# ZJULiHongxin/HRNet-Hand-Pose-Estimation

Measured on AMD Instinct MI355X. Metric: images/sec fwd+bwd pose_hrnet_w32 256x256 bs=64/GPU, higher is better.
Workload: dtype bf16; 1 GPU; pose_hrnet_w32 256x256 bf16 fwd+HeatmapLoss+bwd+Adam training step, batch 64/GPU, synthetic RHD-shaped crops, random-init weights; global_batch=64, parallelism=dp1

## Files before the change

### hrnet-hand-pose-estimation_amd/csrc/loss.hip

```cpp
#include "common.h"

namespace {

__device__ __forceinline__ float block_sum(float v, float* red) {
  v = wave_sum64(v);
  const int w = threadIdx.x >> 6;
  if ((threadIdx.x & 63) == 0) red[w] = v;
  __syncthreads();
  float s = 0.f;
  for (int k = 0; k < (int)(blockDim.x >> 6); ++k) s += red[k];
  __syncthreads();
  return s;
}

__device__ __forceinline__ float block_max(float v, float* red) {
#pragma unroll
  for (int o = 32; o > 0; o >>= 1) v = fmaxf(v, __shfl_xor(v, o, 64));
  const int w = threadIdx.x >> 6;
  if ((threadIdx.x & 63) == 0) red[w] = v;
  __syncthreads();
  float m = red[0];
  for (int k = 1; k < (int)(blockDim.x >> 6); ++k) m = fmaxf(m, red[k]);
  __syncthreads();
  return m;
// ... 189 lines not shown
    if (inference_style) {
      u = (float)(idx % W);
      v = (float)(idx / W);
      if (!(mx > 0.f)) u = v = 0.f;
    } else {
      u = (float)(idx % H);
      v = (float)(idx / H);
    }
    preds[blockIdx.x * 2] = u;
    preds[blockIdx.x * 2 + 1] = v;
    if (maxvals) maxvals[blockIdx.x] = mx;
  }
}

__global__ __launch_bounds__(256) void joints_loss_fwd_kernel(const float* pred, const float* gt,
                                                              const float* vis, float* loss, int B, int K) {
  __shared__ float red[4];
  float s = 0.f, sv = 0.f;
  for (int i = threadIdx.x; i < B * K; i += 256) {
    const float dx = pred[2 * i] - gt[2 * i], dy = pred[2 * i + 1] - gt[2 * i + 1];
    const float nrm = sqrtf(dx * dx + dy * dy);
    const float w = vis ? vis[i] : 1.f;
    s = fmaf(nrm, w, s);
    sv += w;
  }
  s = block_sum(s, red);
  sv = block_sum(sv, red);
  if (threadIdx.x == 0) loss[0] = vis ? s / fmaxf(1.f, sv) : s / (float)K;
}

__global__ __launch_bounds__(256) void joints_loss_bwd_kernel(const float* pred, const float* gt,
                                                              const float* vis, const float* gout,
                                                              float* dpred, int B, int K) {
  __shared__ float red[4];
  float sv = 0.f;
  if (vis)
    for (int i = threadIdx.x; i < B * K; i += 256) sv += vis[i];
  sv = block_sum(sv, red);
  const float denom = vis ? fmaxf(1.f, sv) : (float)K;
  const float g = gout[0] / denom;
  for (int i = threadIdx.x; i < B * K; i += 256) {
    const float dx = pred[2 * i] - gt[2 * i], dy = pred[2 * i + 1] - gt[2 * i + 1];
    const float nrm = sqrtf(dx * dx + dy * dy);
    const float w = (vis ? vis[i] : 1.f) * g;
    dpred[2 * i] = nrm > 0.f ? w * dx / nrm : 0.f;
    dpred[2 * i + 1] = nrm > 0.f ? w * dy / nrm : 0.f;
  }
}

__global__ __launch_bounds__(256) void joints3d_loss_fwd_kernel(const float* __restrict__ pred,
                                                                const float* __restrict__ gt,
                                                                float* __restrict__ loss, int B, int K) {
  __shared__ double part[256];
  double s = 0.0;
  for (int i = threadIdx.x; i < B * K; i += 256) {
    const double dx = (double)gt[3 * i] - (double)pred[3 * i], dy = (double)gt[3 * i + 1] - (double)pred[3 * i + 1],
                 dz = (double)gt[3 * i + 2] - (double)pred[3 * i + 2];
    s += sqrt(dx * dx + dy * dy + dz * dz);
  }
  part[threadIdx.x] = s;
  __syncthreads();
  if (threadIdx.x == 0) {
    double total = 0.0;
    for (int i = 0; i < 256; ++i) total += part[i];
    loss[0] = (float)(total / (double)K);
  }
}

__global__ __launch_bounds__(256) void joints3d_loss_bwd_kernel(const float* __restrict__ pred,
                                                                const float* __restrict__ gt,
                                                                const float* __restrict__ gout,
                                                                float* __restrict__ dpred, int n, int K) {
  const double g = (double)gout[0] / (double)K;
  for (int i = blockIdx.x * 256 + threadIdx.x; i < n; i += gridDim.x * 256) {
    const double dx = (double)pred[3 * i] - (double)gt[3 * i], dy = (double)pred[3 * i + 1] - (double)gt[3 * i + 1],
                 dz = (double)pred[3 * i + 2] - (double)gt[3 * i + 2];
    const double nrm = sqrt(dx * dx + dy * dy + dz * dz);
    dpred[3 * i] = nrm == 0.0 ? 0.f : (float)(g * dx / nrm);
    dpred[3 * i + 1] = nrm == 0.0 ? 0.f : (float)(g * dy / nrm);
    dpred[3 * i + 2] = nrm == 0.0 ? 0.f : (float)(g * dz / nrm);
  }
}

__global__ __launch_bounds__(256) void adam_kernel(float* p, const float* g, float* m, float* v,
                                                   long long n, float lr, float b1, float b2, float eps,
                                                   float wd, float bc1, float bc2_sqrt, float gscale) {
  for (long long i = (long long)blockIdx.x * blockDim.x + threadIdx.x; i < n;
       i += (long long)gridDim.x * blockDim.x) {
    float gi = g[i] * gscale;
    const float pi = p[i];
    gi = fmaf(wd, pi, gi);
    const float mi = b1 * m[i] + (1.f - b1) * gi;
    const float vi = b2 * v[i] + (1.f - b2) * gi * gi;
    m[i] = mi;
    v[i] = vi;
    const float denom = sqrtf(vi) / bc2_sqrt + eps;
    p[i] = pi - (lr / bc1) * (mi / denom);
  }
}

constexpr int kHandJoints = 21;
constexpr int kStructThreads = 256;

__device__ __forceinline__ double hand_scale(double (&x)[kHandJoints][2]) {
  const double wx = x[0][0], wy = x[0][1];
#pragma unroll
  for (int j = 0; j < kHandJoints; ++j) {
    x[j][0] -= wx;
    x[j][1] -= wy;
  }
  const double ux = x[9][0] - x[0][0], uy = x[9][1] - x[0][1];
  const double s = sqrt(ux * ux + uy * uy);
#pragma unroll
  for (int j = 0; j < kHandJoints; ++j) {
    x[j][0] /= s;
    x[j][1] /= s;
  }
  return s;
}

__device__ __forceinline__ void hand_grad_store(double (&g)[kHandJoints][2], const double (&x)[kHandJoints][2],
                                                double s, int normalize, float* __restrict__ out) {
  if (normalize) {
    double gs = 0.0;
#pragma unroll
    for (int j = 0; j < kHandJoints; ++j) {
      gs += g[j][0] * x[j][0] + g[j][1] * x[j][1];
      g[j][0] /= s;
      g[j][1] /= s;
    }
    gs = -gs / s;
    const double ux = x[9][0] - x[0][0], uy = x[9][1] - x[0][1];
    const double nx = s == 0.0 ? 0.0 : ux, ny = s == 0.0 ? 0.0 : uy;
    g[9][0] += gs * nx;
    g[9][1] += gs * ny;
    g[0][0] -= gs * nx;
    g[0][1] -= gs * ny;
    double sx = 0.0, sy = 0.0;
#pragma unroll
    for (int j = 0; j < kHandJoints; ++j) {
      sx += g[j][0];
      sy += g[j][1];
    }
    g[0][0] -= sx;
    g[0][1] -= sy;
  }
#pragma unroll
  for (int j = 0; j < kHandJoints; ++j) {
    out[2 * j] = (float)g[j][0];
    out[2 * j + 1] = (float)g[j][1];
  }
}

__device__ __forceinline__ void hand_load(const float* __restrict__ p, double (&x)[kHandJoints][2]) {
#pragma unroll
  for (int j = 0; j < kHandJoints; ++j) {
    x[j][0] = (double)p[2 * j];
    x[j][1] = (double)p[2 * j + 1];
  }
}

__global__ __launch_bounds__(kStructThreads) void structure_loss_kernel(const float* __restrict__ pred,
                                                                        const float* __restrict__ gt,
                                                                        float* __restrict__ loss_bone,
                                                                        float* __restrict__ loss_angle,
                                                                        float* __restrict__ dbone,
                                                                        float* __restrict__ dangle, int B,
                                                                        int normalize, int terms) {
  __shared__ double part[2][kStructThreads];
  double sum_bone = 0.0, sum_angle = 0.0;
  for (int base = 0; base < B; base += kStructThreads) {
    const int b = base + (int)threadIdx.x;
    double lb = 0.0, la = 0.0;
    if (b < B) {
      double x[kHandJoints][2], g[kHandJoints][2];
      hand_load(pred + (size_t)b * kHandJoints * 2, x);
      const double s = normalize ? hand_scale(x) : 1.0;
      if (terms & 1) {
        double lg[kHandJoints];
        {
// ... 181 lines not shown
extern "C" int hrnet_decode_argmax(const float* hms, float* preds, float* maxvals, int BK, int H, int W,
                                   int inference_style, hr_stream_t stream) {
  HR_REQUIRE(hms && preds && BK > 0 && H > 0 && W > 0, "decode_argmax: args");
  hipLaunchKernelGGL(decode_argmax_kernel, dim3(BK), dim3(256), 0, (hipStream_t)stream, hms, preds,
                     maxvals, H, W, inference_style);
  return hr_check_launch("decode_argmax");
}

extern "C" int hrnet_joints_loss_fwd(const float* pred, const float* gt, const float* vis, float* loss,
                                     int B, int K, hr_stream_t stream) {
  HR_REQUIRE(pred && gt && loss && B > 0 && K > 0, "joints_loss_fwd: args");
  hipLaunchKernelGGL(joints_loss_fwd_kernel, dim3(1), dim3(256), 0, (hipStream_t)stream, pred, gt, vis,
                     loss, B, K);
  return hr_check_launch("joints_loss_fwd");
}

extern "C" int hrnet_joints_loss_bwd(const float* pred, const float* gt, const float* vis,
                                     const float* gout, float* dpred, int B, int K, hr_stream_t stream) {
  HR_REQUIRE(pred && gt && gout && dpred && B > 0 && K > 0, "joints_loss_bwd: args");
  hipLaunchKernelGGL(joints_loss_bwd_kernel, dim3(1), dim3(256), 0, (hipStream_t)stream, pred, gt, vis,
                     gout, dpred, B, K);
  return hr_check_launch("joints_loss_bwd");
}

extern "C" int hrnet_joints3d_loss_fwd(const float* pred, const float* gt, float* loss, int B, int K,
                                       hr_stream_t stream) {
  HR_REQUIRE(pred && gt && loss && B > 0 && K > 0 && (long long)B * K <= (1LL << 28), "joints3d_loss_fwd: args");
  hipLaunchKernelGGL(joints3d_loss_fwd_kernel, dim3(1), dim3(256), 0, (hipStream_t)stream, pred, gt, loss, B, K);
  return hr_check_launch("joints3d_loss_fwd");
}

extern "C" int hrnet_joints3d_loss_bwd(const float* pred, const float* gt, const float* gout, float* dpred, int B,
                                       int K, hr_stream_t stream) {
  HR_REQUIRE(pred && gt && gout && dpred && B > 0 && K > 0 && (long long)B * K <= (1LL << 28),
             "joints3d_loss_bwd: args");
  const int n = B * K;
  int grid = (n + 255) / 256;
  if (grid > 1024) grid = 1024;
  hipLaunchKernelGGL(joints3d_loss_bwd_kernel, dim3((unsigned)grid), dim3(256), 0, (hipStream_t)stream, pred, gt,
                     gout, dpred, n, K);
  return hr_check_launch("joints3d_loss_bwd");
}

extern "C" int hrnet_structure_loss(const float* pred, const float* gt, float* loss_bone, float* loss_angle,
                                    float* dbone_dpred, float* dangle_dpred, int B, int K, int normalize, int terms,
                                    hr_stream_t stream) {
  HR_REQUIRE(pred && B > 0, "structure_loss: args");
  HR_REQUIRE(K == kHandJoints, "structure_loss: K must be 21 (the hand skeleton of the reference's losses)");
  HR_REQUIRE(terms >= 1 && terms <= 3, "structure_loss: terms is a mask of 1 (bone length) and 2 (joint angle)");
  HR_REQUIRE(!(terms & 1) || (gt && loss_bone), "structure_loss: the bone-length term needs gt and loss_bone");
  HR_REQUIRE(!(terms & 2) || loss_angle, "structure_loss: the joint-angle term needs loss_angle");
  hipLaunchKernelGGL(structure_loss_kernel, dim3(1), dim3(kStructThreads), 0, (hipStream_t)stream, pred, gt,
                     loss_bone, loss_angle, (terms & 1) ? dbone_dpred : nullptr, (terms & 2) ? dangle_dpred : nullptr,
                     B, normalize ? 1 : 0, terms);
  return hr_check_launch("structure_loss");
}

extern "C" int hrnet_structure_loss_bwd(const float* dbone_dpred, const float* dangle_dpred, const float* g_bone,
                                        const float* g_angle, float* dpred, int B, int K, hr_stream_t stream) {
  HR_REQUIRE(dpred && B > 0 && K == kHandJoints, "structure_loss_bwd: args");
  HR_REQUIRE((g_bone || g_angle) && (!g_bone || dbone_dpred) && (!g_angle || dangle_dpred),
             "structure_loss_bwd: an upstream gradient needs its unit gradient");
  const long long n = (long long)B * K * 2;
  long long grid = (n + 255) / 256;
  if (grid > 1024) grid = 1024;
  hipLaunchKernelGGL(structure_loss_bwd_kernel, dim3((unsigned)grid), dim3(256), 0, (hipStream_t)stream,
                     dbone_dpred, dangle_dpred, g_bone, g_angle, dpred, n);
  return hr_check_launch("structure_loss_bwd");
}

extern "C" int hrnet_adam_step(float* param, const float* grad, float* exp_avg, float* exp_avg_sq,
                               int64_t n, float lr, float beta1, float beta2, float eps,
                               float weight_decay, int step, float grad_scale, hr_stream_t stream) {
  HR_REQUIRE(param && grad && exp_avg && exp_avg_sq && n > 0 && step >= 1, "adam_step: args");
  const double bc1 = 1.0 - pow((double)beta1, (double)step);
  const double bc2 = 1.0 - pow((double)beta2, (double)step);
  long long grid = (n + 255) / 256;
  if (grid > 8192) grid = 8192;
  hipLaunchKernelGGL(adam_kernel, dim3((unsigned)grid), dim3(256), 0, (hipStream_t)stream, param, grad,
                     exp_avg, exp_avg_sq, (long long)n, lr, beta1, beta2, eps, weight_decay, (float)bc1,
                     (float)sqrt(bc2), grad_scale);
  return hr_check_launch("adam_step");
}
```

### hrnet-hand-pose-estimation_amd/lib/hipnet/net.py

```python
import torch
import torch.nn as nn

from . import _capi as C
from . import ops
from .engine import BNRec, ConvRec, Plan, Program


class HipNet(object):
    def __init__(self, module, stage_cfg, compute_dtype):
        self.module = module
        self.stage_cfg = stage_cfg
        self.compute_dtype = compute_dtype
        self.dtid = C.dtype_id(compute_dtype)
        C.lib()
        params = list(module.parameters())
        if not params or not params[0].is_cuda:
            raise RuntimeError('pose_hrnet: parameters must live on a HIP device (model.cuda()); '
                               'there is no CPU path')
        self.device = params[0].device
        self.plans = {}
        self.fwd_packed = self.bwd_packed = False
        self._flatten(params)
        self._records()

    def _flatten(self, params):
        names = {id(p): n for n, p in self.module.named_parameters()}
        self._late_ids = {id(p) for p in params if p.requires_grad and self._is_late(names.get(id(p), ''), p)}
        params = ([p for p in params if p.requires_grad and id(p) not in self._late_ids]
                  + [p for p in params if id(p) in self._late_ids] + [p for p in params if not p.requires_grad])
        self.trainable_count = sum(p.numel() for p in params if p.requires_grad)
        self.late_start = sum(p.numel() for p in params if p.requires_grad and id(p) not in self._late_ids)
        total = sum(p.numel() for p in params)
        self.flat_p = torch.empty(total, dtype=torch.float32, device=self.device)
        self.flat_g = torch.zeros(total, dtype=torch.float32, device=self.device)
        self.params = params
        self._gview = {}
        self.offsets = {}
        off = 0
        with torch.no_grad():
            for p in params:
                n = p.numel()
                self.flat_p[off:off + n].copy_(p.detach().reshape(-1).float())
                p.data = self.flat_p[off:off + n].view(p.shape)
                self._gview[id(p)] = self.flat_g[off:off + n].view(p.shape)
                self.offsets[id(p)] = (off, n)
                if p.grad is not None:
                    self._gview[id(p)].copy_(p.grad)
                    p.grad = self._gview[id(p)]
                off += n
        self.total_params = total

    def grad_of(self, p):
        return self._gview[id(p)]

    def layout(self):
        names = {id(p): n for n, p in self.module.named_parameters()}
        return [(names[id(p)],) + self.offsets[id(p)] for p in self.params if p.requires_grad]

    def param_order(self):
        return [n for n, _p in self.module.named_parameters()]

    @staticmethod
    def _is_late(name, p):
        if p.dim() != 4 or not name.startswith('stage') or not name.endswith('.weight'):
            return False
        parts = name.split('.')
        if 'fuse_layers' in parts:
            return True
        return 'branches' in parts and int(parts[parts.index('branches') + 1]) >= 2

    def is_late(self, p):
        return id(p) in self._late_ids

    def _records(self):
        self.convs, self.bns, self.bn_list, self.bias_pad = {}, {}, {}, {}
        self.bn_list = []
        skip = tuple(getattr(self.module, 'hip_skip_prefixes', ()))
        for name, m in self.module.named_modules():
            if skip and name.startswith(skip):
                continue
            if isinstance(m, nn.Conv2d):
                r = ConvRec(name, m, stem=(name == 'conv1'))
                es = torch.empty((), dtype=self.compute_dtype).element_size()
                taps = r.ks * r.ks
                nf = r.Cout_pad * (1 if r.stem else taps) * r.Cin_pad
                r.wf = torch.empty(nf * es, dtype=torch.uint8, device=self.device)
                if not r.stem:
                    r.wd = torch.empty(r.Cin_pad * taps * r.Cout_pad * es, dtype=torch.uint8, device=self.device)
                self.convs[name] = r
                if m.bias is not None:
                    self.bias_pad[name] = torch.zeros(r.Cout_pad, dtype=torch.float32, device=self.device)
            elif isinstance(m, nn.BatchNorm2d):
                b = BNRec(name, m, self.device)
                self.bns[name] = b
                self.bn_list.append(b)
        self.pack_f = self._pack_program([(r, 2 if r.stem else 0, r.wf) for r in self.convs.values()])
        self.pack_d = self._pack_program([(r, 1, r.wd) for r in self.convs.values() if r.wd is not None])

    def _pack_program(self, items):
        import ctypes
        ents = (C.HrPackEnt * len(items))()
        block = 0
        for e, item in zip(ents, items):
            r, mode, out = item[:3]
            taps = r.ks * r.ks
            if (mode == 1 and r.Cout_pad * (taps + 1) > 4864) or (mode == 0 and r.Cin * taps > 4864):
                raise ValueError('{}: {} output channels at {}x{} exceed the LDS staging of the weight packer'.format(
                    r.prefix, r.Cout, r.ks, r.ks))
            e.w, e.out = C.ptr(r.mod.weight), C.ptr(out)
            e.Cout, e.Cin, e.ks, e.Cout_pad, e.Cin_pad, e.mode = r.Cout, r.Cin, r.ks, r.Cout_pad, r.Cin_pad, mode
            if len(item) > 3:
                c0, c = item[3], item[4]
                assert r.ks == 1 and mode == 0
                e.w = r.mod.weight.data_ptr() + 4 * c0
                e.Cin, e.Cin_pad, e.ld = c, c, r.Cin
            e.block0 = block
            block += C.call('hrnet_pack_blocks', e.Cout_pad, e.Cin_pad, r.ks, mode)
        raw = bytes(ctypes.string_at(ctypes.addressof(ents), ctypes.sizeof(ents)))
        table = torch.frombuffer(bytearray(raw), dtype=torch.uint8).to(self.device)
        self._tables = getattr(self, '_tables', []) + [table]
        prog = Program()
        prog.add(ops.make(C.OP_PACK_TABLE, dtype=self.dtid, n=len(items), blocks=block, table=C.ptr(table)))
        return prog.finalize()

    def head_slices(self, crec, widths):
        key = (crec.prefix, tuple(widths))
        if getattr(self, '_head_key', None) != key:
            es = torch.empty((), dtype=self.compute_dtype).element_size()
            items, off = [], 0
            self._head_wf = []
            for c in widths:
                out = torch.empty(crec.Cout_pad * c * es, dtype=torch.uint8, device=self.device)
                self._head_wf.append(out)
                items.append((crec, 0, out, off, c))
                off += c
            self._head_pack = self._pack_program(items)
            self._head_key = key
            self._head_pack.run()
        return self._head_wf

    def pack_weights(self, for_backward):
        if not self.fwd_packed:
            self.pack_f.run()
            if getattr(self, '_head_pack', None) is not None:
                self._head_pack.run()
            for name, buf in self.bias_pad.items():
                b = self.convs[name].mod.bias
                buf[:b.numel()].copy_(b.detach())
            self.fwd_packed = True
        if for_backward and not self.bwd_packed:
            self.pack_d.run()
            self.bwd_packed = True

    def mark_weights_dirty(self):
        self.fwd_packed = self.bwd_packed = False

    MAX_PLANS_IN_FLIGHT = 4

    def plan(self, N, H, W, training, need_grad):
        key = (N, H, W, bool(training), bool(need_grad))
        pool = self.plans.setdefault(key, [])
        for p in pool:
            if not (need_grad and p.busy):
                return p
        if len(pool) >= self.MAX_PLANS_IN_FLIGHT:
            raise RuntimeError('pose_hrnet: {} training forwards of shape {} are waiting for their backward; run '
                               'backward (or drop the outputs) before more forwards'.format(len(pool), (N, H, W)))
        p = Plan(self, N, H, W, training, need_grad)
        pool.append(p)
        return p

    def forward(self, x, training, need_grad):
        if x.dim() != 4 or x.shape[1] != 3:
            raise ValueError('pose_hrnet expects (B,3,H,W) input, got {}'.format(tuple(x.shape)))
        N, _, H, W = x.shape
        if H % 32 or W % 32:
            raise ValueError('pose_hrnet: input height/width must be multiples of 32, got {}x{}'.format(H, W))
        if need_grad and not training:
            raise RuntimeError('pose_hrnet: backward through eval-mode BatchNorm is not implemented')
        self.pack_weights(for_backward=need_grad)
        plan = self.plan(N, H, W, training, need_grad)
        hm, inter = plan.run_forward(x)
        return hm, inter, plan

    def all_plans(self):
        return [p for pool in self.plans.values() for p in pool]

    def prepare_grads(self):
        ours = [p.grad is not None and p.grad.data_ptr() == self._gview[id(p)].data_ptr() for p in self.params]
        if not any(ours):
            foreign = [(p, p.grad) for p in self.params if p.grad is not None]
            self.flat_g.zero_()
            for p, g in foreign:
                self._gview[id(p)].copy_(g)
            for p in self.params:
                p.grad = self._gview[id(p)]
            return
        for p, mine in zip(self.params, ours):
            if p.grad is None:
                self._gview[id(p)].zero_()
                p.grad = self._gview[id(p)]
            elif not mine:
                self._gview[id(p)].copy_(p.grad)
                p.grad = self._gview[id(p)]

    def backward(self, plan, g_hm, g_inter, segment_hook=None):
        self.prepare_grads()
        if segment_hook is not None:
            segment_hook.begin(plan)
        plan.run_backward(g_hm, g_inter, segment_hook)
        self.mark_weights_dirty()
```

### hrnet-hand-pose-estimation_amd/lib/hipnet/optim.py

```python
import torch

from . import _capi as C


class FlatAdam(object):
    def __init__(self, model, lr=1e-3, betas=(0.9, 0.999), eps=1e-8, weight_decay=0.0):
        self.model = model
        self.lr, self.betas, self.eps, self.weight_decay = lr, betas, eps, weight_decay
        self.step_count = 0
        self.grad_scale = 1.0
        self._state_for = None
        self.param_groups = [{'lr': lr, 'initial_lr': lr, 'weight_decay': weight_decay, 'betas': betas, 'eps': eps}]

    def _state(self):
        net = self.model.hip()
        if self._state_for is not net:
            self.exp_avg = torch.zeros_like(net.flat_p)
            self.exp_avg_sq = torch.zeros_like(net.flat_p)
            self._state_for = net
        return net

    def zero_grad(self, set_to_none=True):
        net = self._state()
        if set_to_none:
            for p in net.params:
                p.grad = None
        else:
            net.flat_g.zero_()

    def step(self):
        net = self._state()
        self.step_count += 1
        lr = self.param_groups[0]['lr']
        C.call('hrnet_adam_step', net.flat_p.data_ptr(), net.flat_g.data_ptr(), self.exp_avg.data_ptr(),
               self.exp_avg_sq.data_ptr(), net.trainable_count, lr, self.betas[0], self.betas[1], self.eps,
               self.weight_decay, self.step_count, self.grad_scale, C.stream_ptr())
        net.mark_weights_dirty()

    def state_dict(self):
        net = self._state()
        return {'step': self.step_count, 'exp_avg': self.exp_avg, 'exp_avg_sq': self.exp_avg_sq,
                'param_groups': self.param_groups, 'layout': net.layout()}

    def load_state_dict(self, sd):
        net = self._state()
        cur = net.layout()
        saved = sd.get('layout')
        if saved is None:
            saved = legacy_layout(cur, net.param_order())
        self.step_count = sd['step']
        self.exp_avg.copy_(remap_flat(sd['exp_avg'], saved, cur, self.exp_avg.numel()))
        self.exp_avg_sq.copy_(remap_flat(sd['exp_avg_sq'], saved, cur, self.exp_avg_sq.numel()))
        self.param_groups = sd['param_groups']


def legacy_layout(cur_layout, module_order):
    size = {name: n for name, _o, n in cur_layout}
    out, off = [], 0
    for name in module_order:
        if name in size:
            out.append((name, off, size[name]))
            off += size[name]
    return out


def remap_flat(saved, saved_layout, cur_layout, cur_numel):
    saved_layout = [(str(a), int(b), int(c)) for a, b, c in saved_layout]
    cur_layout = [(str(a), int(b), int(c)) for a, b, c in cur_layout]
    if saved_layout == cur_layout and saved.numel() == cur_numel:
        return saved
    smap = {name: (off, n) for name, off, n in saved_layout}
    if set(smap) != {name for name, _o, _n in cur_layout}:
        missing = sorted({name for name, _o, _n in cur_layout} ^ set(smap))[:5]
        raise ValueError('optimizer checkpoint does not match this model (parameter names differ: {} ...)'.format(missing))
    out = saved.new_zeros(cur_numel)
    for name, off, n in cur_layout:
        so, sn = smap[name]
        if sn != n or so + sn > saved.numel():
            raise ValueError('optimizer checkpoint does not match this model ({}: {} vs {} elements)'.format(name, sn, n))
        out[off:off + n] = saved[so:so + sn]
    return out


class GradSync(object):

    def __init__(self, model, optimizer=None, bucket_bytes=16 << 20, process_group=None, broadcast=True):
        import torch.distributed as dist
        self.dist = dist
        self.pg = process_group
        self.world = dist.get_world_size(process_group)
        self.model = model
        self.bucket_bytes = bucket_bytes
        self.cuts = []
        self._ranges = {}
        self._works = []
        self._plan = None
        self._done = set()
        self.scale_in_finish = True
        model._segment_hook = self
        if optimizer is not None:
            self.attach(optimizer)
        if broadcast:
            self.broadcast_state()

    def attach(self, optimizer):
        if hasattr(optimizer, 'grad_scale'):
            optimizer.grad_scale = 1.0 / self.world
            self.scale_in_finish = False
        else:
            self.scale_in_finish = True

    def broadcast_state(self, src=0):
        net = self.model.hip()
        self.dist.broadcast(net.flat_p, src, group=self.pg)
        for b in self.model.buffers():
            self.dist.broadcast(b, src, group=self.pg)
# ... 119 lines not shown
```

### include/hrnet_hip.h

```cpp
#ifndef HRNET_HIP_H
#define HRNET_HIP_H

#include <stdint.h>

#ifdef __cplusplus
extern "C" {
#endif

#define HR_ABI_VERSION 2
#define HR_HOST

typedef void* hr_stream_t;
typedef int hr_value_t;

enum { HR_F32 = 0, HR_BF16 = 1 };

enum {
  HR_OK = 0,
  HR_E_BADARG = -1,
  HR_E_LAUNCH = -2,
  HR_E_BADOP = -3
};

enum {
// ... 459 lines not shown
enum { HR_TF_ACT_NONE = 0, HR_TF_ACT_GELU = 1 };
hr_value_t hrnet_tf_supported(int op, int a, int b);
long long hrnet_tf_layernorm_scratch(long long rows, int C);
int hrnet_tf_layernorm(const float* x, const float* gamma, const float* beta, float* y, long long rows, int C, float eps,
                       hr_stream_t stream);
int hrnet_tf_layernorm_bwd(const float* x, const float* gamma, const float* dy, float* dx, float* dgamma, float* dbeta,
                           float* scratch, long long scratch_floats, long long rows, int C, float eps,
                           hr_stream_t stream);
int hrnet_tf_linear(const float* x, const float* W, const float* bias, const float* res, const float* row_scale,
                    float* y, float* pre, long long rows, int Cin, int Cout, int act, hr_stream_t stream);
int hrnet_tf_linear_bwd(const float* x, const float* W, const float* dy, const float* pre, const float* row_scale,
                        float* dx, float* dW, float* db, long long rows, int Cin, int Cout, int act,
                        hr_stream_t stream);
int hrnet_tf_attention(const float* qkv, float* out, int S, int N, int heads, int hd, float scale, hr_stream_t stream);
int hrnet_tf_attention_bwd(const float* qkv, const float* dout, float* dqkv, int S, int N, int heads, int hd,
                           float scale, hr_stream_t stream);
int hrnet_tf_frame_mean(const float* x, const float* w, const float* b, float* y, long long S, int F, long long D,
                        hr_stream_t stream);
int hrnet_tf_frame_mean_bwd(const float* x, const float* w, const float* dy, float* dx, float* dw, float* db,
                            long long S, int F, long long D, hr_stream_t stream);
int hrnet_tf_add_rows(const float* x, const float* pos, float* y, long long rows, int C, int period,
                      hr_stream_t stream);

enum { HR_SWIN_ATTENTION = 0, HR_SWIN_MERGE = 1, HR_SWIN_EMBED = 2 };
hr_value_t hrnet_swin_supported(int op, int a, int b);
int hrnet_swin_attention(const float* qkv, const float* qkv_bias, const float* bias_table, float* out, int B, int H,
                         int W, int heads, int hd, int ws, int shift, float scale, hr_stream_t stream);
int hrnet_swin_merge_ln(const float* x, const float* gamma, const float* beta, float* y, int B, int H, int W, int C,
                        float eps, hr_stream_t stream);
int hrnet_swin_patch_rows(const float* x, float* rows, int B, int Cin, int H, int W, int p, hr_stream_t stream);

hr_value_t hrnet_swin_attention_bwd_scratch(int B, int H, int W, int heads, int hd, int ws);
int hrnet_swin_attention_bwd(const float* qkv, const float* qkv_bias, const float* bias_table, const float* dout,
                             float* dqkv, float* dqkv_bias, float* dtable, float* scratch, long long scratch_floats,
                             int B, int H, int W, int heads, int hd, int ws, int shift, float scale, hr_stream_t stream);
int hrnet_swin_merge_scatter(const float* dy, float* dx, int B, int H, int W, int C, hr_stream_t stream);
int hrnet_swin_patch_rows_bwd(const float* drows, float* dx, int B, int Cin, int H, int W, int p, hr_stream_t stream);
int hrnet_swin_deconv_dgrad(const float* du, const float* w_packed, float* dx, int B, int H, int W, int Cout_p, int Cin_p,
                            hr_stream_t stream);

enum { HR_NMF_UPDATE = 0, HR_NMF_GRAM = 1, HR_NMF_PRODUCT = 2 };
hr_value_t hrnet_nmf_supported(int op, int a, int b);
int hrnet_nmf_update(const float* T, const float* F, const float* x, long long ldx, long long bsx, int xt, const float* Gm,
                     float* Tout, int G, int M, int K, int R, float eps, hr_stream_t stream);
hr_value_t hrnet_nmf_gram_scratch(int G, int K, int R);
int hrnet_nmf_gram(const float* A, float* Gm, float* scratch, long long scratch_floats, int G, int K, int R,
                   hr_stream_t stream);
int hrnet_nmf_product(const float* x, long long ldx, long long bsx, int xt, const float* F, float* out, int G, int M, int K,
                      int R, hr_stream_t stream);
int hrnet_nmf_reconstruct(const float* Bs, const float* Cf, float* out, long long ldo, long long bso, int ot, int G, int D,
                          int N, int R, hr_stream_t stream);

int hrnet_burger_mix(const float* u, const float* s, const float* coef_ham, const float* coef_shortcut, float* out,
                     long long rows, int C, hr_stream_t stream);
hr_value_t hrnet_burger_mix_scratch(long long rows, int C);
int hrnet_burger_mix_bwd(const float* g, const float* out, const float* u, const float* s, const float* coef_ham,
                         const float* coef_shortcut, float* du, float* ds, float* dcoef, double* scratch,
                         long long scratch_doubles, long long rows, int C, hr_stream_t stream);
int hrnet_dropout2d(const float* x, const float* keep, float* y, int B, long long P, int C, hr_stream_t stream);

int hrnet_spatial_softmax_fwd(const float* x, const float* temp, float* out, int BK, int HW,
                              hr_stream_t stream);
int hrnet_spatial_softmax_bwd(const float* x, const float* out, const float* gout, const float* temp,
                              float* dx, float* dtemp_partial, int BK, int HW, hr_stream_t stream);

int hrnet_joints_loss_fwd(const float* pred, const float* gt, const float* vis, float* loss, int B,
                          int K, hr_stream_t stream);
int hrnet_joints_loss_bwd(const float* pred, const float* gt, const float* vis, const float* gout,
                          float* dpred, int B, int K, hr_stream_t stream);

int hrnet_joints3d_loss_fwd(const float* pred, const float* gt, float* loss, int B, int K, hr_stream_t stream);
int hrnet_joints3d_loss_bwd(const float* pred, const float* gt, const float* gout, float* dpred, int B, int K,
                            hr_stream_t stream);

int hrnet_structure_loss(const float* pred, const float* gt, float* loss_bone, float* loss_angle,
                         float* dbone_dpred, float* dangle_dpred, int B, int K, int normalize, int terms,
                         hr_stream_t stream);
int hrnet_structure_loss_bwd(const float* dbone_dpred, const float* dangle_dpred, const float* g_bone,
                             const float* g_angle, float* dpred, int B, int K, hr_stream_t stream);

int hrnet_adam_step(float* param, const float* grad, float* exp_avg, float* exp_avg_sq, int64_t n,
                    float lr, float beta1, float beta2, float eps, float weight_decay, int step,
                    float grad_scale, hr_stream_t stream);

int hrnet_deform_conv_forward(const float* input, const float* offset, const float* weight,
                              const float* bias, float* output, int B, int C, int H, int W, int Co,
                              int kh, int kw, int sh, int sw, int ph, int pw, int dh, int dw,
                              int groups, int deformable_groups, hr_stream_t stream);
hr_value_t hrnet_deform_conv_wgrad_blocks(int B, int Ho, int Wo);
int hrnet_deform_conv_backward(const float* input, const float* offset, const float* weight,
                               const float* grad_output, float* grad_input, float* grad_offset,
                               float* grad_weight, float* grad_bias, float* scratch, int B, int C,
                               int H, int W, int Co, int kh, int kw, int sh, int sw, int ph, int pw,
                               int dh, int dw, int groups, int deformable_groups,
                               hr_stream_t stream);

int hrnet_modulated_deform_conv_forward(const float* input, const float* offset, const float* mask,
                                        const float* weight, const float* bias, float* output, int B, int C,
                                        int H, int W, int Co, int kh, int kw, int sh, int sw, int ph, int pw,
                                        int dh, int dw, int groups, int deformable_groups, hr_stream_t stream);
int hrnet_modulated_deform_conv_backward(const float* input, const float* offset, const float* mask,
                                         const float* weight, const float* grad_output, float* grad_input,
                                         float* grad_offset, float* grad_mask, float* grad_weight,
                                         float* grad_bias, float* scratch, int B, int C, int H, int W, int Co,
                                         int kh, int kw, int sh, int sw, int ph, int pw, int dh, int dw,
                                         int groups, int deformable_groups, hr_stream_t stream);

int hrnet_conv2d_kxk(int dtype, const void* x, const void* w, const float* bias, void* y, int N, int H, int W, int Cin,
                     int ldx, int x_off, int Cout, int ldy, int y_off, int ks, int relu, hr_stream_t stream);
hr_value_t hrnet_conv_kxk_tile(int which);
int hrnet_maxpool2d_3x3s2(const float* x, float* y, int N, int H, int W, int C, int ldx, int x_off, int ldy, int y_off,
                          hr_stream_t stream);
int hrnet_avgpool2d_9s8(const float* x, float* y, int N, int H, int W, int ldy, int y_off, hr_stream_t stream);

int hrnet_conv2d_kxk_wgrad_scratch(int dtype, int N, int H, int W, int Cin, int Cout, int ks, HR_HOST long long* bytes,
                                   HR_HOST int* nsplit, HR_HOST long long* split_tiles);
int hrnet_conv2d_kxk_wgrad(int dtype, const void* x, const void* dy, void* scratch, long long scratch_bytes, float* dw,
                           float* db, int N, int H, int W, int Cin, int Cin_real, int ldx, int x_off, int Cout, int ldy,
                           int y_off, int ks, hr_stream_t stream);
int hrnet_conv2d_kxk_dgrad(int dtype, const void* dy, const void* wT, void* dx, const float* mask, int N, int H, int W,
                           int Cout, int ldy, int y_off, int Cin, int ldx, int x_off, int ldm, int m_off, int ks,
                           int accumulate, hr_stream_t stream);
int hrnet_maxpool2d_3x3s2_bwd(const float* x, const float* dy, float* dx, int N, int H, int W, int C, int ldx, int x_off,
                              int lddy, int dy_off, int lddx, int dx_off, int relu_mask, hr_stream_t stream);

int hrnet_ftl_gather(const float* x, const float* coef, float* y, int B, int V, int H, int W, int C, int ldx, int x_off,
                     int ldy, int y_off, int slice, hr_stream_t stream);
int hrnet_ftl_scatter(const float* f, const float* coef, float* y, int B, int V, int H, int W, int C, int ldf, int f_off,
                      int ldy, int y_off, hr_stream_t stream);
int hrnet_conv2d_3x3g(int dtype, const void* x, const void* w, const float* bias, void* y, int N, int H, int W, int Cin,
                      int ldx, int x_off, int Cout, int ldy, int y_off, int Ho, int Wo, int stride, int pad_lo, int z,
                      int relu, hr_stream_t stream);

int hrnet_ftl_gather_bwd(const float* dcat, const float* coef, float* dx, int B, int V, int H, int W, int C, int ldd,
                         int d_off, int slice, int ldx, int x_off, hr_stream_t stream);
int hrnet_ftl_scatter_bwd(const float* dy, const float* coef, float* df, int B, int V, int H, int W, int C, int ldy,
                          int y_off, int ldf, int f_off, hr_stream_t stream);
int hrnet_conv2d_3x3g_wgrad_scratch(int dtype, int N, int Ho, int Wo, int Cin, int Cout, HR_HOST long long* bytes,
                                    HR_HOST int* nsplit, HR_HOST long long* split_tiles);
int hrnet_conv2d_3x3g_wgrad(int dtype, const void* x, const void* dy, void* scratch, long long scratch_bytes, float* dw,
                            int N, int H, int W, int Cin, int Cin_real, int ldx, int x_off, int Cout, int ldy, int y_off,
                            int Ho, int Wo, int stride, int pad_lo, hr_stream_t stream);

int hrnet_upsample_slice_nchw(const float* src, float* dst, int N, int h, int w, int Cp, int c0, int C,
                              int H, int W, hr_stream_t stream);
int hrnet_upsample_slice_nchw_bwd(const float* ddst, float* dsrc, int N, int h, int w, int Cp, int c0, int C,
                                  int H, int W, int accumulate, hr_stream_t stream);
hr_value_t hrnet_upsample_slice_nchw_supported(int Cp, int c0, int C);

int hrnet_sample_stats_scratch(int B, long long n0, long long n1, long long n2, HR_HOST long long* bytes);
int hrnet_sample_stats(const float* x0, const float* x1, const float* x2, long long n0, long long n1, long long n2, int B,
                       double eps, void* scratch, long long scratch_bytes, float* stats, hr_stream_t stream);
int hrnet_stlstm_gates(const float* xc, const float* hc, const float* mc, const float* stats, const float* wx,
                       const float* bx, const float* wh, const float* bh, const float* wm, const float* bm,
                       const float* c_t, int ldc, int c_off, const float* m_t, int ldmt, int m_off, float* mem, int ldmem,
                       float* o_pre, int B, int H, int W, int nh, hr_stream_t stream);
int hrnet_stlstm_out(const float* oc, const float* stats, const float* wo, const float* bo, const float* o_pre,
                     const float* last, float* h_new, int B, int H, int W, int nh, hr_stream_t stream);
int hrnet_maxpool2d_2x2(const float* x, float* y, int N, int H, int W, int C, int ldx, int x_off, int ldy, int y_off,
                        hr_stream_t stream);

#ifdef __cplusplus
}
#endif
#endif
```

Measured before the change: 4327 images/sec.

## Fuse Adam update with bf16 conv weight packing into one kernel

Adds an Adam kernel that, for each conv weight, updates the fp32 master params and at the same time writes the packed compute-dtype forward weights, plus the transposed backward weights once backward has run. The intent is to skip the separate weight-packing passes after every optimizer step, which re-read the whole flat parameter buffer. The Adam math is wrapped in a shared helper with FP contraction turned off so the fused and plain paths round the same way. It relies on a per-entry block table built on the host and falls back to the plain path when alignment or layout checks fail.

```diff
diff --git a/hrnet-hand-pose-estimation_amd/csrc/loss.hip b/hrnet-hand-pose-estimation_amd/csrc/loss.hip
--- a/hrnet-hand-pose-estimation_amd/csrc/loss.hip
+++ b/hrnet-hand-pose-estimation_amd/csrc/loss.hip
@@ -295,20 +295,182 @@
   }
 }
 
+__device__ __forceinline__ float adam_update(float pi, float g, float& m, float& v, float lr, float b1, float b2,
+                                             float eps, float wd, float bc1, float bc2_sqrt, float gscale) {
+#pragma clang fp contract(off)
+  float gi = g * gscale;
+  gi = fmaf(wd, pi, gi);
+  const float mi = b1 * m + (1.f - b1) * gi;
+  const float vi = b2 * v + (1.f - b2) * gi * gi;
+  m = mi;
+  v = vi;
+  const float denom = sqrtf(vi) / bc2_sqrt + eps;
+  return fmaf(-(lr / bc1), mi / denom, pi);
+}
+
 __global__ __launch_bounds__(256) void adam_kernel(float* p, const float* g, float* m, float* v,
                                                    long long n, float lr, float b1, float b2, float eps,
                                                    float wd, float bc1, float bc2_sqrt, float gscale) {
   for (long long i = (long long)blockIdx.x * blockDim.x + threadIdx.x; i < n;
        i += (long long)gridDim.x * blockDim.x) {
-    float gi = g[i] * gscale;
-    const float pi = p[i];
-    gi = fmaf(wd, pi, gi);
-    const float mi = b1 * m[i] + (1.f - b1) * gi;
-    const float vi = b2 * v[i] + (1.f - b2) * gi * gi;
+    float mi = m[i], vi = v[i];
+    const float pn = adam_update(p[i], g[i], mi, vi, lr, b1, b2, eps, wd, bc1, bc2_sqrt, gscale);
     m[i] = mi;
     v[i] = vi;
-    const float denom = sqrtf(vi) / bc2_sqrt + eps;
-    p[i] = pi - (lr / bc1) * (mi / denom);
+    p[i] = pn;
+  }
+}
+
+constexpr int AP_CO = 32;
+constexpr int AP_ROW = 288;
+constexpr int AP_PITCH = AP_ROW + 1;
+constexpr int AP_PLAIN = 1024;
+
+__host__ __device__ inline int adam_pack_cit(int taps, int mode) {
+  if (mode == 2) return AP_ROW / taps;
+  for (int c = 256; c >= 8; c >>= 1)
+    if (c * taps <= AP_ROW) return c;
+  return 0;
+}
+
+struct AdamPackArgs {
+  float* p;
+  const float* g;
+  float* m;
+  float* v;
+  const HrPackEnt* tab;
+  void* const* out_t;
+  const int32_t* block_entry;
+  int with_t;
+  float lr, b1, b2, eps, wd, bc1, bc2_sqrt, gscale;
+};
+
+__device__ __forceinline__ float adam_pack_update(const AdamPackArgs& a, float pi, float g, float& m, float& v) {
+  return adam_update(pi, g, m, v, a.lr, a.b1, a.b2, a.eps, a.wd, a.bc1, a.bc2_sqrt, a.gscale);
+}
+
+template <typename T>
+__global__ __launch_bounds__(256) void adam_pack_kernel(AdamPackArgs a) {
+  constexpr int VEC = TT<T>::VEC;
+  __shared__ float buf[AP_CO * AP_PITCH];
+  const int tid = threadIdx.x;
+  const int ent = a.block_entry[blockIdx.x];
+  const HrPackEnt e = a.tab[ent];
+  const int u = (int)blockIdx.x - e.block0;
+  const long long base = (const float*)e.w - (const float*)a.p;
+  if (e.mode == 3) {
+    const long long lo = base + (long long)u * AP_PLAIN + tid, hi = base + e.Cin;
+    float pv[4], gv[4], mv[4], vv[4];
+#pragma unroll
+    for (int k = 0; k < 4; ++k) {
+      const long long i = lo + k * 256;
+      if (i < hi) { pv[k] = a.p[i]; gv[k] = a.g[i]; mv[k] = a.m[i]; vv[k] = a.v[i]; }
+    }
+#pragma unroll
+    for (int k = 0; k < 4; ++k) {
+      const long long i = lo + k * 256;
+      if (i < hi) {
+        const float pn = adam_pack_update(a, pv[k], gv[k], mv[k], vv[k]);
+        a.m[i] = mv[k]; a.v[i] = vv[k]; a.p[i] = pn;
+      }
+    }
+    return;
+  }
+  const int taps = e.ks * e.ks;
+  const int cit = adam_pack_cit(taps, e.mode);
+  const int ncit = e.mode == 2 ? 1 : (e.Cin_pad + cit - 1) / cit;
+  const int cot = u / ncit, cib = u - cot * ncit;
+  const int co0 = cot * AP_CO, ci0 = cib * cit;
+  const int rows_pad = e.Cout_pad - co0 < AP_CO ? e.Cout_pad - co0 : AP_CO;
+  const int rows_real = e.Cout - co0 < AP_CO ? e.Cout - co0 : AP_CO;
+  const int cw_real = e.Cin - ci0 < cit ? e.Cin - ci0 : cit;
+  const int len = cw_real * taps;
+  if (rows_real > 0 && len > 0) {
+    const long long a0 = base + ((long long)co0 * e.Cin + ci0) * taps;
+    const long long rstride = (long long)e.Cin * taps;
+    const int nv = (len + 3) / 4 + 1;
+    int r = tid / nv, j = tid - r * nv;
+    const int dr = 256 / nv, dj = 256 - dr * nv;
+    while (r < rows_real) {
+      const long long ar = a0 + r * rstride;
+      const long long i0 = ((ar >> 2) + j) << 2;
+      const int rel = (int)(i0 - ar);
+      float* row = buf + r * AP_PITCH;
+      if (rel >= 0 && rel + 4 <= len) {
+        const f32x4 pv = *(const f32x4*)(a.p + i0), gv = *(const f32x4*)(a.g + i0);
+        const f32x4 mv = *(const f32x4*)(a.m + i0), vv = *(const f32x4*)(a.v + i0);
+        float m0 = mv.x, m1 = mv.y, m2 = mv.z, m3 = mv.w, v0 = vv.x, v1 = vv.y, v2 = vv.z, v3 = vv.w;
+        f32x4 pn;
+        pn.x = adam_pack_update(a, pv.x, gv.x, m0, v0);
+        pn.y = adam_pack_update(a, pv.y, gv.y, m1, v1);
+        pn.z = adam_pack_update(a, pv.z, gv.z, m2, v2);
+        pn.w = adam_pack_update(a, pv.w, gv.w, m3, v3);
+        *(f32x4*)(a.m + i0) = f32x4{m0, m1, m2, m3};
+        *(f32x4*)(a.v + i0) = f32x4{v0, v1, v2, v3};
+        *(f32x4*)(a.p + i0) = pn;
+        row[rel] = pn.x; row[rel + 1] = pn.y; row[rel + 2] = pn.z; row[rel + 3] = pn.w;
+      } else if (rel > -4 && rel < len) {
+#pragma unroll
+        for (int k = 0; k < 4; ++k)
+          if (rel + k >= 0 && rel + k < len) {
+            const long long i = i0 + k;
+            float mi = a.m[i], vi = a.v[i];
+            const float pn = adam_pack_update(a, a.p[i], a.g[i], mi, vi);
+            a.m[i] = mi; a.v[i] = vi; a.p[i] = pn;
+            row[rel + k] = pn;
+          }
+      }
+      r += dr; j += dj;
+      if (j >= nv) { j -= nv; ++r; }
+    }
+  }
+  __syncthreads();
+  T* of = (T*)e.out;
+  if (e.mode == 2) {
+    const int nvec = e.Cin_pad / VEC, kreal = taps * e.Cin;
+    for (int i = tid; i < rows_pad * nvec; i += 256) {
+      const int r = i / nvec, k0 = (i - r * nvec) * VEC;
+      float f[VEC];
+#pragma unroll
+      for (int k = 0; k < VEC; ++k) {
+        const int kk = k0 + k, t = kk / e.Cin, ci = kk - t * e.Cin;
+        f[k] = (r < rows_real && kk < kreal) ? buf[r * AP_PITCH + ci * taps + t] : 0.f;
+      }
+      *(V16*)(of + (size_t)(co0 + r) * e.Cin_pad + k0) = v16_pack<T>(f);
+    }
+    return;
+  }
+  const int cwp = e.Cin_pad - ci0 < cit ? e.Cin_pad - ci0 : cit;
+  {
+    const int nvec = cwp / VEC, nrt = rows_pad * taps;
+    int rt = tid / nvec, vq = tid - rt * nvec;
+    const int dr = 256 / nvec, dj = 256 - dr * nvec;
+    while (rt < nrt) {
+      const int r = rt / taps, t = rt - r * taps, c = vq * VEC;
+      const float* src = buf + r * AP_PITCH + c * taps + t;
+      float f[VEC];
+#pragma unroll
+      for (int k = 0; k < VEC; ++k) f[k] = (r < rows_real && c + k < cw_real) ? src[k * taps] : 0.f;
+      *(V16*)(of + ((size_t)(co0 + r) * taps + t) * e.Cin_pad + ci0 + c) = v16_pack<T>(f);
+      rt += dr; vq += dj;
+      if (vq >= nvec) { vq -= nvec; ++rt; }
+    }
+  }
+  T* ot = a.with_t ? (T*)a.out_t[ent] : nullptr;
+  if (ot != nullptr) {
+    const int nvec = rows_pad / VEC, nct = cwp * taps;
+    int ct = tid / nvec, vq = tid - ct * nvec;
+    const int dr = 256 / nvec, dj = 256 - dr * nvec;
+    while (ct < nct) {
+      const int cl = ct / taps, tf = ct - cl * taps, r0 = vq * VEC;
+      const float* src = buf + r0 * AP_PITCH + cl * taps + (taps - 1 - tf);
+      float f[VEC];
+#pragma unroll
+      for (int k = 0; k < VEC; ++k) f[k] = (r0 + k < rows_real && cl < cw_real) ? src[k * AP_PITCH] : 0.f;
+      *(V16*)(ot + ((size_t)(ci0 + cl) * taps + tf) * e.Cout_pad + co0 + r0) = v16_pack<T>(f);
+      ct += dr; vq += dj;
+      if (vq >= nvec) { vq -= nvec; ++ct; }
+    }
   }
 }
 
@@ -656,3 +818,35 @@
                      (float)sqrt(bc2), grad_scale);
   return hr_check_launch("adam_step");
 }
+
+extern "C" int hrnet_adam_pack_blocks(int Cout_pad, int Cin_pad, int ks, int mode) {
+  if (mode == 3) return Cin_pad > 0 ? (Cin_pad + AP_PLAIN - 1) / AP_PLAIN : 0;
+  if ((mode != 0 && mode != 2) || ks < 1 || Cout_pad < 16 || Cout_pad % 16 || Cin_pad < 8 || Cin_pad % 8) return 0;
+  const int cit = adam_pack_cit(ks * ks, mode);
+  if (cit < 1) return 0;
+  const int cot = (Cout_pad + AP_CO - 1) / AP_CO;
+  return mode == 2 ? cot : cot * ((Cin_pad + cit - 1) / cit);
+}
+
+extern "C" int hrnet_adam_pack_step(int dtype, float* param, const float* grad, float* exp_avg, float* exp_avg_sq,
+                                    const HrPackEnt* table, const void* out_t, const int32_t* block_entry,
+                                    int total_blocks, int with_t, float lr, float beta1, float beta2, float eps,
+                                    float weight_decay, int step, float grad_scale, hr_stream_t stream) {
+  HR_REQUIRE(param && grad && exp_avg && exp_avg_sq && table && out_t && block_entry && total_blocks >= 1 &&
+                 step >= 1, "adam_pack_step: args");
+  HR_REQUIRE((((uintptr_t)param | (uintptr_t)grad | (uintptr_t)exp_avg | (uintptr_t)exp_avg_sq) & 15) == 0,
+             "adam_pack_step: the flat buffers must be 16-byte aligned");
+  HR_REQUIRE(dtype == HR_F32 || dtype == HR_BF16, "adam_pack_step: dtype");
+  const double bc1 = 1.0 - pow((double)beta1, (double)step);
+  const double bc2 = 1.0 - pow((double)beta2, (double)step);
+  AdamPackArgs a;
+  a.p = param; a.g = grad; a.m = exp_avg; a.v = exp_avg_sq;
+  a.tab = table; a.out_t = (void* const*)out_t; a.block_entry = block_entry; a.with_t = with_t;
+  a.lr = lr; a.b1 = beta1; a.b2 = beta2; a.eps = eps; a.wd = weight_decay;
+  a.bc1 = (float)bc1; a.bc2_sqrt = (float)sqrt(bc2); a.gscale = grad_scale;
+  if (dtype == HR_F32)
+    hipLaunchKernelGGL(adam_pack_kernel<float>, dim3((unsigned)total_blocks), dim3(256), 0, (hipStream_t)stream, a);
+  else
+    hipLaunchKernelGGL(adam_pack_kernel<bf16_t>, dim3((unsigned)total_blocks), dim3(256), 0, (hipStream_t)stream, a);
+  return hr_check_launch("adam_pack_step");
+}
diff --git a/hrnet-hand-pose-estimation_amd/lib/hipnet/net.py b/hrnet-hand-pose-estimation_amd/lib/hipnet/net.py
--- a/hrnet-hand-pose-estimation_amd/lib/hipnet/net.py
+++ b/hrnet-hand-pose-estimation_amd/lib/hipnet/net.py
@@ -19,7 +19,8 @@
                                'there is no CPU path')
         self.device = params[0].device
         self.plans = {}
-        self.fwd_packed = self.bwd_packed = False
+        self.fwd_packed = self.bwd_packed = self.aux_packed = False
+        self.bwd_ever = False
         self._flatten(params)
         self._records()
 
@@ -142,18 +143,87 @@
     def pack_weights(self, for_backward):
         if not self.fwd_packed:
             self.pack_f.run()
+            self.fwd_packed = True
+        if not self.aux_packed:
             if getattr(self, '_head_pack', None) is not None:
                 self._head_pack.run()
             for name, buf in self.bias_pad.items():
                 b = self.convs[name].mod.bias
                 buf[:b.numel()].copy_(b.detach())
-            self.fwd_packed = True
-        if for_backward and not self.bwd_packed:
-            self.pack_d.run()
-            self.bwd_packed = True
+            self.aux_packed = True
+        if for_backward:
+            self.bwd_ever = True
+            if not self.bwd_packed:
+                self.pack_d.run()
+                self.bwd_packed = True
 
     def mark_weights_dirty(self):
-        self.fwd_packed = self.bwd_packed = False
+        self.fwd_packed = self.bwd_packed = self.aux_packed = False
+
+    def mark_convs_packed(self, with_t):
+        self.fwd_packed = True
+        self.bwd_packed = bool(with_t)
+        self.aux_packed = False
+
+    def adam_pack_table(self):
+        if not hasattr(self, '_adam_pack'):
+            self._adam_pack = self._build_adam_pack()
+        return self._adam_pack
+
+    def _build_adam_pack(self):
+        import ctypes
+        from .engine import _knob
+        if _knob('HRNET_ADAM_PACK', '1') == '0' or self.compute_dtype not in (torch.float32, torch.bfloat16):
+            return None
+        if self.flat_p.data_ptr() % 16 or self.flat_g.data_ptr() % 16 or not self.convs:
+            return None
+        by_off = {}
+        for r in self.convs.values():
+            w = r.mod.weight
+            off, n = self.offsets[id(w)]
+            if not w.requires_grad or off + n > self.trainable_count or off in by_off:
+                return None
+            if r.stem and r.Cin * r.ks * r.ks > min(288, r.Cin_pad):
+                return None
+            by_off[off] = r
+        items, pos = [], 0
+        for p in self.params:
+            off, n = self.offsets[id(p)]
+            if not p.requires_grad or n == 0:
+                continue
+            assert off == pos, 'the flat buffer is not [trainable | frozen]'
+            pos = off + n
+            r = by_off.get(off)
+            if r is None and items and items[-1][2] is None and items[-1][1] + n < (1 << 31):
+                items[-1] = (items[-1][0], items[-1][1] + n, None)
+            else:
+                items.append((off, n, r))
+        if pos != self.trainable_count:
+            return None
+        ents = (C.HrPackEnt * len(items))()
+        out_t = torch.zeros(len(items), dtype=torch.int64)
+        counts, block = [], 0
+        for k, (e, (off, n, r)) in enumerate(zip(ents, items)):
+            e.w = self.flat_p.data_ptr() + 4 * off
+            if r is None:
+                e.Cin, e.mode = n, 3
+                nb = C.call('hrnet_adam_pack_blocks', 0, n, 1, 3)
+            else:
+                e.out = C.ptr(r.wf)
+                e.Cout, e.Cin, e.ks, e.Cout_pad, e.Cin_pad = r.Cout, r.Cin, r.ks, r.Cout_pad, r.Cin_pad
+                e.mode = 2 if r.stem else 0
+                out_t[k] = C.ptr(r.wd) if r.wd is not None else 0
+                nb = C.call('hrnet_adam_pack_blocks', r.Cout_pad, r.Cin_pad, r.ks, e.mode)
+            if nb < 1:
+                return None
+            e.block0 = block
+            counts.append(nb)
+            block += nb
+        raw = bytes(ctypes.string_at(ctypes.addressof(ents), ctypes.sizeof(ents)))
+        table = torch.frombuffer(bytearray(raw), dtype=torch.uint8).to(self.device)
+        block_entry = torch.repeat_interleave(torch.arange(len(items), dtype=torch.int32),
+                                              torch.tensor(counts)).to(self.device)
+        return table, out_t.to(self.device), block_entry, block
 
     MAX_PLANS_IN_FLIGHT = 4
 
diff --git a/hrnet-hand-pose-estimation_amd/lib/hipnet/optim.py b/hrnet-hand-pose-estimation_amd/lib/hipnet/optim.py
--- a/hrnet-hand-pose-estimation_amd/lib/hipnet/optim.py
+++ b/hrnet-hand-pose-estimation_amd/lib/hipnet/optim.py
@@ -32,6 +32,16 @@
         net = self._state()
         self.step_count += 1
         lr = self.param_groups[0]['lr']
+        fused = net.adam_pack_table() if hasattr(net, 'adam_pack_table') else None
+        if fused is not None and self.exp_avg.data_ptr() % 16 == 0 and self.exp_avg_sq.data_ptr() % 16 == 0:
+            table, out_t, block_entry, blocks = fused
+            with_t = 1 if net.bwd_ever else 0
+            C.call('hrnet_adam_pack_step', net.dtid, net.flat_p.data_ptr(), net.flat_g.data_ptr(),
+                   self.exp_avg.data_ptr(), self.exp_avg_sq.data_ptr(), table.data_ptr(), out_t.data_ptr(),
+                   block_entry.data_ptr(), blocks, with_t, lr, self.betas[0], self.betas[1], self.eps,
+                   self.weight_decay, self.step_count, self.grad_scale, C.stream_ptr())
+            net.mark_convs_packed(with_t)
+            return
         C.call('hrnet_adam_step', net.flat_p.data_ptr(), net.flat_g.data_ptr(), self.exp_avg.data_ptr(),
                self.exp_avg_sq.data_ptr(), net.trainable_count, lr, self.betas[0], self.betas[1], self.eps,
                self.weight_decay, self.step_count, self.grad_scale, C.stream_ptr())
diff --git a/include/hrnet_hip.h b/include/hrnet_hip.h
--- a/include/hrnet_hip.h
+++ b/include/hrnet_hip.h
@@ -565,6 +565,11 @@
 int hrnet_adam_step(float* param, const float* grad, float* exp_avg, float* exp_avg_sq, int64_t n,
                     float lr, float beta1, float beta2, float eps, float weight_decay, int step,
                     float grad_scale, hr_stream_t stream);
+int hrnet_adam_pack_step(int dtype, float* param, const float* grad, float* exp_avg, float* exp_avg_sq,
+                         const HrPackEnt* table, const void* out_t, const int32_t* block_entry, int total_blocks,
+                         int with_t, float lr, float beta1, float beta2, float eps, float weight_decay, int step,
+                         float grad_scale, hr_stream_t stream);
+hr_value_t hrnet_adam_pack_blocks(int Cout_pad, int Cin_pad, int ks, int mode);
 
 int hrnet_deform_conv_forward(const float* input, const float* offset, const float* weight,
                               const float* bias, float* output, int B, int C, int H, int W, int Co,
```

Result: no change. 4347 images/sec, median of 6 (+0.5%).
